# dzufferey/round

Hardware: AMD Instinct MI355X
Metric: checked process-rounds/sec (node), OTR n=64 w/ invariants; % HBM peak (higher is better)
Workload: dtype int32

## Files before the change

round_amd/csrc/psg_api.hip:

```cpp
#include <hip/hip_runtime.h>

#include <algorithm>
#include <cstdio>
#include <cstdlib>
#include <cstring>
#include <new>
#include <string>
#include <thread>
#include <utility>
#include <vector>

#include "../../include/psg.h"
#include "psg_device.hpp"
#include "psg_kernels.hpp"

namespace psg {

__global__ void gen_init_kernel(uint64_t inst_begin, uint64_t count, int n, int alg, int V, uint64_t seed,
                                int32_t* out) {
  const uint64_t total = count * (uint64_t)n;
  for (uint64_t e = (uint64_t)blockIdx.x * blockDim.x + threadIdx.x; e < total; e += (uint64_t)gridDim.x * blockDim.x) {
    const uint64_t i = e / (uint64_t)n;
    const int p = (int)(e - i * (uint64_t)n);
    const uint64_t w = rword(seed, inst_begin + i, ROUND_INIT, (uint32_t)p, 0);
// ... 81 lines not shown
  bool init_f64_host = false;
  std::string module_path;
  hipModule_t module = nullptr;
  hipFunction_t native_fn = nullptr;
  hipFunction_t fused_fn = nullptr, fused_x_fn = nullptr;
  int32_t module_alg = 0;
  bool staged = false;
  bool staged_host = false;
  uint64_t staged_begin = 0, staged_count = 0;
  bool ho_loaded = false, ho_has_crash = false;
  bool pop_crash = false;
  uint64_t ho_begin = 0, ho_count = 0;
  uint64_t last_count = 0;
  int grid_max = 0;
  std::string err;
  std::vector<psg_ctx*> subs;
};

static thread_local std::string g_create_err;

static const char* const k_names_otr[] = {"Safety", "Invariant0", "Invariant1", "Invariant2",
                                          "Agreement", "Validity", "Integrity", "Irrevocability"};
static const char* const k_names_lv[] = {"Safety", "Invariant0", "Invariant1", "Agreement",
                                         "Validity", "Integrity", "Irrevocability"};
static const char* const k_names_benor[] = {"Safety", "Invariant0", "Agreement", "Irrevocability", "SafetyPredicate"};
static const char* const k_names_k[] = {"KAgreement", "KValidity"};
static const char* const k_names_eps[] = {"EpsAgreement", "EpsValidity", "SafetyPredicate"};
static const char* const k_names_tpc[] = {"Safety", "Invariant0", "UniformAgreement", "Validity"};
static const char* const k_names_lattice[] = {"Safety", "Invariant0", "Comparability", "DownwardValidity", "UpwardValidity",
                                              "Irrevocability"};
static_assert(std::size(k_names_otr) == kOtrChecks, "k_names_otr and kOtrChecks disagree");
static_assert(std::size(k_names_lv) == kLvChecks, "k_names_lv and kLvChecks disagree");
static_assert(std::size(k_names_benor) == kBenOrChecks, "k_names_benor and kBenOrChecks disagree");
static_assert(std::size(k_names_k) == kKAgreeChecks, "k_names_k and kKAgreeChecks disagree");
static_assert(std::size(k_names_eps) == kEpsilonChecks, "k_names_eps and kEpsilonChecks disagree");
static_assert(std::size(k_names_tpc) == kTpcChecks, "k_names_tpc and kTpcChecks disagree");
static_assert(std::size(k_names_lattice) == kLatticeChecks, "k_names_lattice and kLatticeChecks disagree");

struct CheckNames {
  const char* const* name;
  int count;
  constexpr CheckNames() : name(nullptr), count(0) {}
  template <int N>
  constexpr CheckNames(const char* const (&a)[N]) : name(a), count(N) {}
};

struct AlgRow {
  const char* class_name;
  CheckNames checks;
  void (*defaults)(psg_config& cfg, int n);
  const char* (*invalid)(const psg_config& cfg);
  hipError_t (*launch)(const KArgs& a, int W, int grid, hipStream_t s);
  const void* (*kernel)(int W);
};

static const char* need_value_range(const psg_config& c) { return c.value_range < 1 ? "value_range must be >= 1" : nullptr; }

static void lv_defaults(psg_config& c, int n) {
  c.value_range = (1 << 15) - 1;
  c.sched.drop_log2 = 4;
  c.sched.good_p32 = 0;
  c.sched.crash_fmax = (n - 1) / 2;
}

static void crash_stop_defaults(psg_config& c, int rounds, int fmax) {
  c.param = 2;
  c.rounds = rounds;
  c.value_range = 1000000;
  c.sched.drop_log2 = 0;
  c.sched.good_p32 = 0;
  c.sched.crash_fmax = fmax;
}

static const char* otr_invalid(const psg_config& c) {
  if (const char* m = need_value_range(c)) return m;
  return c.param < 1 ? "OTR needs afterDecision >= 1" : nullptr;
}

static const AlgRow k_algs[] = {
    {},
    {"example.OTR", k_names_otr, [](psg_config& c, int) { c.param = 2;  }, otr_invalid,
     launch_otr, otr_kernel_ptr},
    {"example.LastVoting", k_names_lv, lv_defaults, need_value_range, launch_lv, lv_kernel_ptr},
    {"example.FloodMin", k_names_k, [](psg_config& c, int) { crash_stop_defaults(c, 4, 2); },
     [](const psg_config& c) {
       if (const char* m = need_value_range(c)) return m;
       return c.param < 0 ? "FloodMin needs f >= 0" : nullptr;
     },
     launch_floodmin, floodmin_kernel_ptr},
    {"example.KSetAgreement", k_names_k, [](psg_config& c, int) { crash_stop_defaults(c, 16, 1); },
     [](const psg_config& c) {
       if (const char* m = need_value_range(c)) return m;
       return c.param < 1 ? "KSetAgreement needs k >= 1" : nullptr;
     },
     launch_kset, kset_kernel_ptr},
    {"example.BenOr", k_names_benor,
     [](psg_config& c, int n) {
       c.rounds = 64;
       c.value_range = 2;
       c.sched.drop_log2 = 2;
       c.sched.good_p32 = 0;
       c.sched.ho_min = n / 2;
     },
     [](const psg_config&) -> const char* { return nullptr; }, launch_benor, benor_kernel_ptr},
    {"example.OTR2", k_names_otr, [](psg_config& c, int) { c.param = 2;  }, otr_invalid,
     launch_otr2, otr2_kernel_ptr},
    {"example.ShortLastVoting", k_names_k,
     [](psg_config& c, int n) {
       lv_defaults(c, n);
       c.rounds = 30;
     },
     need_value_range, launch_slv, slv_kernel_ptr},
    {"example.KSetEarlyStopping", k_names_k,
     [](psg_config& c, int) {
       crash_stop_defaults(c, 3, 2);
       c.param2 = 2;
     },
     [](const psg_config& c) {
       if (const char* m = need_value_range(c)) return m;
       return c.param < 0 || c.param2 < 1 ? "KSetEarlyStopping needs t >= 0 and k >= 1" : nullptr;
     },
     launch_kset_es, kset_es_kernel_ptr},
    {"example.EpsilonConsensus", k_names_eps,
     [](psg_config& c, int n) {
       c.param = 1;
       c.real_param = 0.1;
       c.rounds = 12;
       c.sched.drop_log2 = 4;
       c.sched.good_p32 = 0;
       c.sched.ho_min = n - 2;
     },
     [](const psg_config& c) {
       return c.param < 1 || !(c.real_param > 0.0) ? "EpsilonConsensus needs f >= 1 and epsilon > 0" : nullptr;
     },
     launch_epsilon, epsilon_kernel_ptr},
    {"example.TwoPhaseCommit", k_names_tpc,
     [](psg_config& c, int n) {
       c.param = 0;
       c.rounds = 3;
       c.value_range = 2 * n;
       c.sched.drop_log2 = 6;
       c.sched.good_p32 = 0;
     },
     [](const psg_config& c) {
       if (const char* m = need_value_range(c)) return m;
       return c.param < 0 || c.param >= c.n ? "TwoPhaseCommit needs 0 <= coord < n" : nullptr;
     },
     launch_tpc, tpc_kernel_ptr},
    {"example.LatticeAgreement", k_names_lattice,
     [](psg_config& c, int) {
       c.rounds = 8;
       c.value_range = 16;
       c.sched.drop_log2 = 2;
       c.sched.good_p32 = 0;
     },
     [](const psg_config& c) -> const char* {
       return c.value_range < 1 || c.value_range > 31 ? "LatticeAgreement needs 1 <= value_range <= 31" : nullptr;
     },
     launch_lattice, lattice_kernel_ptr},
// ... 346 lines not shown
    sc.batch_capacity = (cfg->batch_capacity + nd - 1) / nd;
    psg_ctx* sub = nullptr;
    const int rc = psg_create(&sub, &sc);
    if (rc) {
      g_create_err = "device " + std::to_string(cfg->devices[d]) + ": " + g_create_err;
      psg_destroy(c);
      return rc;
    }
    c->subs.push_back(sub);
  }
  *out = c;
  return PSG_OK;
}

int psg_create(psg_ctx** out, const psg_config* cfg) {
  if (!out) return PSG_EINVAL;
  *out = nullptr;
  std::string m;
  int rc = validate(cfg, m);
  if (rc) { g_create_err = m; return rc; }
  if (cfg->n_devices > 0) return create_multi(out, cfg);
  int ndev = 0;
  hipError_t e = hipGetDeviceCount(&ndev);
  if (e != hipSuccess || ndev <= 0) { g_create_err = "no HIP device"; return PSG_ENODEV; }
  if (cfg->device < 0 || cfg->device >= ndev) { g_create_err = "device ordinal out of range"; return PSG_ENODEV; }
  psg_ctx* c = new (std::nothrow) psg_ctx();
  if (!c) return PSG_ENOMEM;
  c->cfg = *cfg;
  c->W = (cfg->n + 63) / 64;
  c->cap = cfg->batch_capacity;
  auto bail = [&](hipError_t err, const char* what) {
    g_create_err = std::string(what) + ": " + hipGetErrorString(err);
    psg_destroy(c);
    return err == hipErrorOutOfMemory ? PSG_ENOMEM : PSG_EIO;
  };
#define CK(call) do { hipError_t e_ = (call); if (e_ != hipSuccess) return bail(e_, #call); } while (0)
  CK(hipSetDevice(cfg->device));
  CK(hipStreamCreateWithFlags(&c->stream, hipStreamNonBlocking));
  CK(hipEventCreate(&c->ev0));
  CK(hipEventCreate(&c->ev1));
  const uint64_t cells = c->cap * (uint64_t)cfg->n;
  if (cfg->alg == PSG_ALG_EPSILON) {
    CK(c->d_init_f64.grow(cells));
    CK(c->d_dec_f64.grow(cells));
  } else {
    CK(c->d_init.grow(cells));
  }
  CK(c->d_dec.grow(cells));
  CK(c->d_dround.grow(cells));
  CK(c->d_inst.grow(c->cap));
  CK(c->d_counters.grow(NCOUNTERS_ALLOC));
  if (cfg->alg == PSG_ALG_KSET && c->W > 1)
    CK(c->d_hand.grow(65 * c->cap + (cells + 1) / 2));
  int per_cu = 0;
  CK(hipOccupancyMaxActiveBlocksPerMultiprocessor(&per_cu, alg_row(cfg->alg)->kernel(c->W), threads_per_block(c->W), 0));
  hipDeviceProp_t prop;
  CK(hipGetDeviceProperties(&prop, cfg->device));
  if (per_cu < 1) per_cu = 1;
  c->grid_max = prop.multiProcessorCount * per_cu;
#undef CK
  *out = c;
  return PSG_OK;
}

static int multi_load_inputs(psg_ctx* c, uint64_t inst_begin, uint64_t count, const int32_t* host_init,
                             const double* host_f64, bool f64) {
  if (count > c->cap) return fail(c, PSG_ERANGE, "inst_count exceeds batch_capacity");
  const uint64_t n = (uint64_t)c->cfg.n, nd = c->subs.size();
  const int rc = par_subs(c, [&](size_t d) {
    uint64_t off, m;
    split(count, nd, d, off, m);
    return f64 ? psg_load_inputs_f64(c->subs[d], inst_begin + off, m, host_f64 ? host_f64 + off * n : nullptr)
               : psg_load_inputs(c->subs[d], inst_begin + off, m, host_init ? host_init + off * n : nullptr);
  });
  if (rc) return rc;
  set_staged(c, inst_begin, count, f64 ? host_f64 != nullptr : host_init != nullptr);
  return PSG_OK;
}

int psg_load_inputs(psg_ctx* c, uint64_t inst_begin, uint64_t count, const int32_t* host_init) {
  if (!c) return PSG_EINVAL;
  if (!c->subs.empty()) {
    if (c->cfg.alg == PSG_ALG_EPSILON && host_init)
      return fail(c, PSG_EINVAL, "EpsilonConsensus takes Double inputs: use psg_load_inputs_f64");
    return multi_load_inputs(c, inst_begin, count, host_init, nullptr, c->cfg.alg == PSG_ALG_EPSILON);
  }
  if (count > c->cap) return fail(c, PSG_ERANGE, "inst_count exceeds batch_capacity");
  if (c->cfg.alg == PSG_ALG_EPSILON) {
    if (host_init) return fail(c, PSG_EINVAL, "EpsilonConsensus takes Double inputs: use psg_load_inputs_f64");
    return psg_load_inputs_f64(c, inst_begin, count, nullptr);
  }
  HIPCHK(c, hipSetDevice(c->cfg.device));
  const uint64_t cells = count * (uint64_t)c->cfg.n;
  if (host_init) {
    HIPCHK(c, hipMemcpyAsync(c->d_init, host_init, sizeof(int32_t) * cells, hipMemcpyHostToDevice, c->stream));
  } else {
    HIPCHK(c, launch_gen_init(inst_begin, count, c->cfg.n, c->cfg.alg, c->cfg.value_range, c->cfg.seed, c->d_init,
                              c->stream));
  }
  HIPCHK(c, hipStreamSynchronize(c->stream));
  set_staged(c, inst_begin, count, host_init != nullptr);
  return PSG_OK;
}

int psg_load_inputs_f64(psg_ctx* c, uint64_t inst_begin, uint64_t count, const double* host_init) {
  if (!c) return PSG_EINVAL;
  if (c->cfg.alg != PSG_ALG_EPSILON) return fail(c, PSG_EINVAL, "Double inputs are for EpsilonConsensus only");
  if (!c->subs.empty()) return multi_load_inputs(c, inst_begin, count, nullptr, host_init, true);
// ... 826 lines not shown
```

round_amd/csrc/psg_device.hpp:

```cpp
#pragma once

#ifndef __HIPCC_RTC__
#include <hip/hip_runtime.h>
#include <stdint.h>
#else
using __hip_internal::int8_t;
using __hip_internal::int16_t;
using __hip_internal::int32_t;
using __hip_internal::int64_t;
using __hip_internal::uint8_t;
using __hip_internal::uint16_t;
using __hip_internal::uint32_t;
using __hip_internal::uint64_t;
#define INT32_MIN (-2147483647 - 1)
#define INT32_MAX 2147483647
#define INT64_MIN (-9223372036854775807LL - 1)
#define INT64_MAX 9223372036854775807LL
#endif

#include "../../include/psg.h"

#define PSG_DEV __device__ __forceinline__

namespace psg {

template <int K>
struct Slot {
  static constexpr int value = K;
};

struct KArgs {
  uint64_t inst_begin;
  uint64_t count;
  const uint64_t* ids;
  const int32_t* init;
  int32_t* out_decision;
  uint8_t* out_dround;
  psg_instance_summary* out_inst;
  psg_process_record* out_rec;
  unsigned long long* counters;
  uint64_t seed;
  const double* init_f64;
  double* out_dec_f64;
  double* out_rec_f64;
  double real_param;
  int32_t* trace;
  uint32_t trace_fields;
  int32_t n, R, V, param, param2, variant, tiebreak;
  uint32_t drop_log2, good_p32;
  int32_t good_min, crash_fmax, ho_min;
  uint32_t self_bit;
  const uint64_t* ho_in;
  const int32_t* crash_in;
  uint64_t ho_base;
  uint64_t init_base;
  uint64_t* hand_hdr;
  uint64_t* hand_meta;
  int32_t* hand_dec;
};

PSG_DEV uint64_t instance_id(const KArgs& a, uint64_t i) { return a.ids ? a.ids[i] : a.inst_begin + i; }
PSG_DEV uint64_t init_row(const KArgs& a, uint64_t i, uint64_t inst) { return a.ids ? inst - a.init_base : i; }
PSG_DEV int32_t init_x(const KArgs& a, uint64_t i, uint64_t inst, int pid) {
#if defined(__HIP_DEVICE_COMPILE__)
  asm volatile("" : "+v"(pid));
#endif
  return a.init[init_row(a, i, inst) * (uint64_t)a.n + (uint64_t)pid];
}

struct VmArgs {
  const int32_t* code;
  const int32_t* slot_entry;
  const int32_t* slot_flags;
  int32_t n_slots, term_entry, n_words;
  const int32_t* trace;
  uint64_t count;
  int32_t n, R;
  psg_instance_summary* out_inst;
  unsigned long long* counters;
  int32_t* err;
};

struct PopArgs {
  uint64_t* ho;
  const uint64_t* src;
  int32_t* init;
  const int32_t* src_init;
  const uint32_t* parent;
  const uint8_t* op;
  uint64_t count;
  int n, R, W;
  uint64_t seed;
  uint32_t gen, flips;
  int32_t min_size;
  uint32_t self_bit;
  uint32_t keep[4];
  int32_t V;
  uint32_t redraw;
  int init_kind;
  int32_t* crash;
  const int32_t* src_crash;
  uint64_t* partial;
  const uint64_t* src_partial;
  int32_t fmax;
  uint32_t partial_p[4];
  uint32_t t_move, t_add, t_drop;
  int32_t live_kind, live_rounds, phase, coord;
  int32_t live_at[PSG_POP_MAX_LIVE];
};
struct LiveArgs {
  const uint64_t* ho;
  uint8_t* live;
  uint64_t count;
  int n, R, W;
  int32_t kind, phase, coord;
};
enum { POP_INIT_VALUE = 0, POP_INIT_COIN = 1, POP_INIT_VOTE = 2, POP_INIT_SET = 3 };

#ifndef PSG_PHASE_TIMERS
#define PSG_PHASE_TIMERS 0
#endif
enum { C_FAIL = 0, C_DECIDED = PSG_MAX_CHECKS, C_DIGEST = PSG_MAX_CHECKS + 1,
       C_ACTIVE = PSG_MAX_CHECKS + 2,
       C_LIVE = PSG_MAX_CHECKS + 3,
       C_HIST = PSG_MAX_CHECKS + 4,
       NCOUNTERS = C_HIST + PSG_MAX_ROUNDS + 2,
       C_QUEUE = NCOUNTERS, NQUEUES = 8, QUEUE_STRIDE = 16, NQUEUE_REGIONS = 2,
       C_TIMER = C_QUEUE + NQUEUE_REGIONS * NQUEUES * QUEUE_STRIDE, NTIMERS = 8, NSTAMP_WAVES = 16384,
       T_RT_SUM = NTIMERS, T_RT_MIN = NTIMERS + 1, T_RT_MAX = NTIMERS + 2, T_WAVES = NTIMERS + 3,
       T_STAMPS = NTIMERS + 4,
       NTIMER_SLOTS = PSG_PHASE_TIMERS ? T_STAMPS + 2 * NSTAMP_WAVES : 0, NCOUNTERS_ALLOC = C_TIMER + NTIMER_SLOTS };

struct PhaseTimers {
#if PSG_PHASE_TIMERS
  uint64_t last, rt0, acc[NTIMERS];
  PSG_DEV void start() {
    for (int j = 0; j < NTIMERS; ++j) acc[j] = 0;
    rt0 = __builtin_amdgcn_s_memrealtime();
    last = __builtin_amdgcn_s_memtime();
  }
  PSG_DEV void mark(int j) {
#if PSG_PHASE_TIMERS == 1
    const uint64_t t = __builtin_amdgcn_s_memtime();
    acc[j] += t - last;
    last = t;
#endif
  }
  PSG_DEV void add(int j, uint64_t v) {
#if PSG_PHASE_TIMERS == 2
    acc[j] += v;
#endif
  }
  PSG_DEV void flush(unsigned long long* g, int lane) {
    const uint64_t rt1 = __builtin_amdgcn_s_memrealtime();
    if (lane == 0) {
      for (int j = 0; j < NTIMERS; ++j) atomicAdd(&g[C_TIMER + j], (unsigned long long)acc[j]);
      atomicAdd(&g[C_TIMER + T_RT_SUM], (unsigned long long)(rt1 - rt0));
      atomicMax(&g[C_TIMER + T_RT_MIN], (unsigned long long)~rt0);
      atomicMax(&g[C_TIMER + T_RT_MAX], (unsigned long long)rt1);
      atomicAdd(&g[C_TIMER + T_WAVES], 1ull);
      const uint32_t wave = blockIdx.x * (blockDim.x >> 6) + (threadIdx.x >> 6);
      if (wave < NSTAMP_WAVES) {
        g[C_TIMER + T_STAMPS + 2 * wave] = rt0;
        g[C_TIMER + T_STAMPS + 1 + 2 * wave] = rt1;
      }
    }
  }
#else
  PSG_DEV void start() {}
  PSG_DEV void mark(int) {}
  PSG_DEV void add(int, uint64_t) {}
  PSG_DEV void flush(unsigned long long*, int) {}
#endif
};

constexpr uint32_t ROUND_INIT = 0xFFFFFFFFu;
constexpr uint32_t ROUND_CRASH = 0xFFFFFFFEu;
constexpr uint32_t PID_GLOBAL = 0xFFFFu;
constexpr uint32_t COIN_TAG = 0x80000000u;

struct U4 { uint32_t x, y, z, w; };

PSG_DEV uint32_t xor3(uint32_t a, uint32_t b, uint32_t c) {
#if defined(__HIP_DEVICE_COMPILE__)
  return __builtin_amdgcn_bitop3_b32(a, b, c, 0x96);
#else
  return a ^ b ^ c;
#endif
}

#ifndef PSG_PHILOX_OPAQUE_KEYS
#define PSG_PHILOX_OPAQUE_KEYS 0
#endif
#ifndef PSG_PHILOX_MAD64
#define PSG_PHILOX_MAD64 2
#endif
#if PSG_PHILOX_MAD64 && defined(__HIP_DEVICE_COMPILE__)
PSG_DEV uint64_t mul64_mad(uint32_t a, uint32_t b) {
  uint64_t r;
#if PSG_PHILOX_MAD64 == 2
  asm("v_mad_u64_u32 %0, vcc, %1, %2, 0" : "=v"(r) : "v"(a), "v"(b) : "vcc");
#else
  uint64_t cy;
  asm("v_mad_u64_u32 %0, %1, %2, %3, 0" : "=v"(r), "=s"(cy) : "v"(a), "v"(b));
#endif
  return r;
}
#define PSG_MUL64(r, a, b) ((r) == 0 ? (uint64_t)(a) * (b) : mul64_mad((a), (b)))
#else
#define PSG_MUL64(r, a, b) ((uint64_t)(a) * (b))
#endif
PSG_DEV U4 philox10(uint32_t c0, uint32_t c1, uint32_t c2, uint32_t c3, uint32_t k0, uint32_t k1) {
#if PSG_PHILOX_OPAQUE_KEYS && defined(__HIP_DEVICE_COMPILE__)
  asm volatile("" : "+s"(k0), "+s"(k1));
#endif
#pragma unroll
  for (int r = 0; r < 10; ++r) {
    const uint64_t p0 = PSG_MUL64(r, 0xD2511F53u, c0);
    const uint64_t p1 = PSG_MUL64(r, 0xCD9E8D57u, c2);
    const uint32_t n0 = xor3((uint32_t)(p1 >> 32), c1, k0);
    const uint32_t n2 = xor3((uint32_t)(p0 >> 32), c3, k1);
    c1 = (uint32_t)p1;
    c3 = (uint32_t)p0;
    c0 = n0;
    c2 = n2;
    k0 += 0x9E3779B9u;
    k1 += 0xBB67AE85u;
  }
  return U4{c0, c1, c2, c3};
}

PSG_DEV uint64_t rword(uint64_t seed, uint64_t inst, uint32_t round, uint32_t ctr3base, uint32_t j) {
  U4 o = philox10((uint32_t)inst, (uint32_t)(inst >> 32), round, ctr3base + ((j >> 1) << 16), (uint32_t)seed,
                  (uint32_t)(seed >> 32));
  return (j & 1u) ? ((uint64_t)o.z | ((uint64_t)o.w << 32)) : ((uint64_t)o.x | ((uint64_t)o.y << 32));
}

struct WordStream {
  uint64_t seed, inst;
  uint32_t round, base;
  int32_t cur;
  uint64_t lo, hi;
  PSG_DEV WordStream(uint64_t s, uint64_t i, uint32_t r, uint32_t b) : seed(s), inst(i), round(r), base(b), cur(-1), lo(0), hi(0) {}
  PSG_DEV uint64_t word(uint32_t j) {
    const int32_t s = (int32_t)(j >> 1);
    if (s != cur) {
      U4 o = philox10((uint32_t)inst, (uint32_t)(inst >> 32), round, base + ((uint32_t)s << 16), (uint32_t)seed,
                      (uint32_t)(seed >> 32));
      lo = (uint64_t)o.x | ((uint64_t)o.y << 32);
      hi = (uint64_t)o.z | ((uint64_t)o.w << 32);
      cur = s;
    }
    return (j & 1u) ? hi : lo;
  }
};

PSG_DEV uint32_t mulhi32(uint32_t a, uint32_t b) { return __umulhi(a, b); }

PSG_DEV int32_t tpc_vote(uint32_t w, uint32_t V) { return mulhi32(w, V) != 0u ? 1 : 0; }

PSG_DEV int32_t lattice_init(uint32_t w, uint32_t U) {
  const uint32_t v = mulhi32(w, U * U);
  return (int32_t)((1u << (v / U)) | (1u << (v % U)));
}

PSG_DEV bool java_first_boolean(uint64_t s) {
  const uint64_t mult = 0x5DEECE66DULL, mask = (1ULL << 48) - 1;
  uint64_t seed = (s ^ mult) & mask;
  seed = (seed * mult + 0xBULL) & mask;
  return (seed >> 47) != 0;
}

PSG_DEV uint32_t scala_improve(uint32_t h) {
  uint32_t x = h + ~(h << 9);
  x ^= (x >> 14);
  x += (x << 4);
  x ^= (x >> 10);
  return x;
}

PSG_DEV uint64_t champ_key(uint32_t h, int depth) {
  uint64_t key = 0;
// ... 505 lines not shown
      return v;
    }
  }
};

template <int W, bool XHO = false>
struct Sched {
  uint64_t seed, inst;
  Mask<W> full;
  int32_t crash_round;
  bool crash_on;
  int good_min, ho_min, V;
  uint32_t drop, good_p32, self_bit;
  int nproc;
  const uint64_t* hop;

  PSG_DEV void setup(const KArgs& args, uint64_t i, int pid, bool valid) {
    hop = nullptr;
    nproc = args.n;
    if constexpr (XHO) {
      const uint64_t row = i - args.ho_base;
      hop = args.ho_in + row * (uint64_t)args.R * (uint64_t)args.n * W;
      seed = args.seed;
      inst = i;
      V = args.V;
      drop = 0;
      good_p32 = 0;
      self_bit = 0;
      ho_min = -1;
      full = mfull<W>(args.n);
      crash_on = false;
      good_min = 0;
      crash_round = (args.crash_in && valid) ? args.crash_in[row * (uint64_t)args.n + pid] : -1;
      return;
    }
    seed = args.seed;
    inst = i;
    V = args.V;
    drop = args.drop_log2;
    good_p32 = args.good_p32;
    self_bit = args.self_bit;
    ho_min = args.ho_min;
    full = mfull<W>(args.n);
    crash_on = args.crash_fmax >= 0;
    good_min = args.good_min >= 0 ? args.good_min : (2 * args.n) / 3;
    crash_round = -1;
    if (crash_on && valid) {
      const uint64_t w0 = rword(seed, i, ROUND_CRASH, PID_GLOBAL, 0);
      const uint64_t w1 = rword(seed, i, ROUND_CRASH, PID_GLOBAL, 1);
      crash_round = crash_of(args, i, (uint32_t)pid, w0, w1);
    }
  }

  PSG_DEV static int32_t crash_of(const KArgs& args, uint64_t i, uint32_t pid, uint64_t w0, uint64_t w1) {
    const uint32_t f = mulhi32((uint32_t)w0, (uint32_t)args.crash_fmax + 1u);
    const uint32_t am = (uint32_t)(w0 >> 32) | 1u;
    const uint32_t off = (uint32_t)w1;
    const uint32_t n = (uint32_t)args.n;
    const bool pow2 = (n & (n - 1)) == 0;
    const uint32_t pos = pow2 ? ((am * pid + off) & (n - 1)) : ((pid + off % n) % n);
    if (pos >= f) return -1;
    return (int32_t)mulhi32((uint32_t)rword(args.seed, i, ROUND_CRASH, pid, 0), (uint32_t)args.R);
  }

  PSG_DEV int32_t init_value(int pid, int alg) const {
    const uint64_t w = rword(seed, inst, ROUND_INIT, (uint32_t)pid, 0);
    if (alg == PSG_ALG_BENOR) return (int32_t)((uint32_t)w & 1u);
    if (alg == PSG_ALG_TPC) return tpc_vote((uint32_t)w, (uint32_t)V);
    if (alg == PSG_ALG_LATTICE) return lattice_init((uint32_t)w, (uint32_t)V);
    return 1 + (int32_t)mulhi32((uint32_t)w, (uint32_t)V);
  }

  PSG_DEV bool coin(int k, int pid) const {
    return java_first_boolean(rword(seed, inst, (uint32_t)k, COIN_TAG | (uint32_t)pid, 0));
  }

  uint64_t good_mask;
  int good_base;
  Mask<W> good_set;

  PSG_DEV void prep_good(int kbase, int lane, int R) {
    good_base = kbase;
    good_mask = 0;
    if (good_p32 == 0) return;
    const int k = kbase + lane;
    WordStream ws(seed, inst, (uint32_t)k, PID_GLOBAL);
    const bool good = k < R && (uint32_t)ws.word(0) < good_p32;
    Mask<W> s = full;
    if (good && drop > 0) {
#pragma unroll
      for (int w = 0; w < W; ++w) {
        uint64_t m = ~0ull;
        for (uint32_t i = 0; i < drop; ++i) m &= ws.word(1u + (uint32_t)w * drop + i);
        s.w[w] &= ~m;
      }
      if (mpopc(s) <= good_min) s = full;
    }
    good_set = s;
    good_mask = __builtin_amdgcn_ballot_w64(good);
  }

  PSG_DEV bool good_round(int k, int lane, int R, Mask<W>& s) {
    if (good_p32 == 0) return false;
    if (k - good_base >= 64) prep_good(k, lane, R);
    const int off = k - good_base;
    const bool good = (good_mask >> off) & 1ull;
// ... 50 lines not shown
      dm[w] = ~0ull;
      hf[w] = ~0ull;
    }
    constexpr bool kSkip = SKIP && W > 1;
    if constexpr (kSkip) {
      if (__builtin_expect(drop == 0 && crash, 0)) {
        {
#pragma unroll
          for (int sc2 = 0; 2 * sc2 < W; ++sc2) {
            if (!((cw >> (2 * sc2)) & 3u)) continue;
            const U4 o = philox10((uint32_t)inst, (uint32_t)(inst >> 32), k, pid + ((uint32_t)sc2 << 16),
                                  (uint32_t)seed, (uint32_t)(seed >> 32));
            hf[2 * sc2] = (uint64_t)o.x | ((uint64_t)o.y << 32);
            if (2 * sc2 + 1 < W) hf[2 * sc2 + 1] = (uint64_t)o.z | ((uint64_t)o.w << 32);
          }
        }
        return;
      }
    }
    draw_words<kSkip>(k, pid, j0, j1, nd, cw, dm, hf);
  }

  PSG_DEV Mask<W> assemble(int pid, bool good, const Mask<W>& goodS, const Mask<W>& CB, const Mask<W>& CN,
                           const uint64_t (&dm)[W], const uint64_t (&hf)[W]) const {
    Mask<W> base;
#pragma unroll
    for (int w = 0; w < W; ++w) {
      base.w[w] = good ? goodS.w[w] : (drop > 0 ? full.w[w] & ~dm[w] : full.w[w]);
      if (crash_on) base.w[w] &= ~(CB.w[w] | (CN.w[w] & ~hf[w]));
    }
    if (self_bit) mset(base, pid);
    if (ho_min >= 0 && mpopc(base) <= ho_min) base = full;
    return base;
  }

  template <bool SKIP = true>
  PSG_DEV Mask<W> ho(int k, int pid, bool good, const Mask<W>& goodS, const Mask<W>& CB, const Mask<W>& CN) const {
    if constexpr (XHO) {
      Mask<W> m = mzero<W>();
      if (pid < nproc) {
        const uint64_t* q = hop + ((uint64_t)k * (uint64_t)nproc + (uint64_t)pid) * W;
#pragma unroll
        for (int w = 0; w < W; ++w) m.w[w] = __builtin_nontemporal_load(q + w) & full.w[w];
      }
      return m;
    }
    uint64_t dm[W], hf[W];
    uint32_t cw = 0;
#pragma unroll
    for (int w = 0; w < W; ++w) cw |= CN.w[w] ? 1u << w : 0u;
    draw<SKIP>((uint32_t)k, (uint32_t)pid, good, crash_on && cw != 0u, dm, hf, cw);
    return assemble(pid, good, goodS, CB, CN, dm, hf);
  }
};

template <int W, bool XHO>
PSG_DEV Mask<W> ho_select(const Sched<W, XHO>& sc, int k, int pid, bool good, const Mask<W>& goodS, const Mask<W>& CB,
                       const Mask<W>& CN) {
  if constexpr (XHO) {
    return sc.ho(k, pid, good, goodS, CB, CN);
  } else {
    uint64_t dm[W], hf[W];
    uint32_t cw = 0;
#pragma unroll
    for (int w = 0; w < W; ++w) cw |= CN.w[w] ? 1u << w : 0u;
    sc.draw((uint32_t)k, (uint32_t)pid, good, sc.crash_on && cw != 0u, dm, hf, cw);
    const uint64_t self = sc.self_bit ? 1ull << (pid & 63) : 0ull;
    Mask<W> base;
#pragma unroll
    for (int w = 0; w < W; ++w) {
      base.w[w] = good ? goodS.w[w] : (sc.drop > 0 ? sc.full.w[w] & ~dm[w] : sc.full.w[w]);
      if (sc.crash_on) base.w[w] &= ~(CB.w[w] | (CN.w[w] & ~hf[w]));
      base.w[w] |= (pid >> 6) == w ? self : 0ull;
    }
    if (sc.ho_min >= 0 && mpopc(base) <= sc.ho_min) base = sc.full;
    return base;
  }
}

template <int W>
struct CrashSets {
  int32_t cr[W];
  PSG_DEV void prep(Grp<W>& g, int32_t* lds, int32_t my_crash_round) {
    if constexpr (W == 1) {
      cr[0] = my_crash_round;
    } else {
      lds[g.pid] = g.valid ? my_crash_round : -1;
      __syncthreads();
#pragma unroll
      for (int w = 0; w < W; ++w) cr[w] = lds[w * 64 + g.lane];
    }
  }
  PSG_DEV void sets(Grp<W>& g, int k, Mask<W>& CB, Mask<W>& CN) const {
    if constexpr (W == 1) {
      CB = g.ballot_any((uint32_t)cr[0] < (uint32_t)k);
      CN = g.ballot_any(cr[0] == k);
    } else {
#pragma unroll
      for (int w = 0; w < W; ++w) {
        CB.w[w] = __builtin_amdgcn_ballot_w64((uint32_t)cr[w] < (uint32_t)k);
        CN.w[w] = __builtin_amdgcn_ballot_w64(cr[w] == k);
      }
    }
  }
};

template <int W, bool XHO>
struct Inst {
  uint64_t id;
  Sched<W, XHO> sc;
  CrashSets<W> cs;
  PSG_DEV void begin(Grp<W>& g, const KArgs& a, uint64_t i, int32_t* crl) {
    begin_front(g, a, i, crl);
    sc.prep_good(0, g.lane, a.R);
  }
  PSG_DEV void begin_front(Grp<W>& g, const KArgs& a, uint64_t i, int32_t* crl) {
    id = instance_id(a, i);
    sc.setup(a, id, g.pid, g.valid);
    if (sc.crash_on) cs.prep(g, crl, sc.crash_round);
  }
  PSG_DEV int32_t x0(const Grp<W>& g, const KArgs& a, uint64_t i, int alg) const {
    if (!g.valid) return 0;
    return a.init ? init_x(a, i, id, g.pid) : sc.init_value(g.pid, alg);
  }
};

struct GoodFront {
  static constexpr int kRows = 8, kRounds = 4, kLate = 32;
  static constexpr uint64_t kNone = 1ull << 63;
  uint64_t g0 = kNone;
  uint32_t set;
  uint32_t mask;
  int base;

  PSG_DEV static bool pass(const Sched<1, false>& sc, uint64_t id, uint32_t k, int lane, int R, uint64_t& s) {
    const uint32_t c = (uint32_t)lane >> 5;
    const U4 o = philox10((uint32_t)id, (uint32_t)(id >> 32), k, PID_GLOBAL + (c << 16), (uint32_t)sc.seed,
                          (uint32_t)(sc.seed >> 32));
    const uint64_t lo = (uint64_t)o.x | ((uint64_t)o.y << 32);
    const uint64_t hi = (uint64_t)o.z | ((uint64_t)o.w << 32);
    const uint64_t t = sc.drop >= 3 ? (lo & hi) : (sc.drop == 2 ? lo : ~0ull);
    const uint64_t up = (uint64_t)xshfl<32>((uint32_t)t, lane) | ((uint64_t)xshfl<32>((uint32_t)(t >> 32), lane) << 32);
    const bool good = lane < 32 && (int)k < R && o.x < sc.good_p32;
    s = sc.full.w[0];
    if (good && sc.drop > 0) {
      uint64_t m = hi & up;
      for (uint32_t c2 = 2; 2 * c2 <= sc.drop; ++c2) {
        const U4 q = philox10((uint32_t)id, (uint32_t)(id >> 32), k, PID_GLOBAL + (c2 << 16), (uint32_t)sc.seed,
                              (uint32_t)(sc.seed >> 32));
        m &= (uint64_t)q.x | ((uint64_t)q.y << 32);
        if (2 * c2 + 1 <= sc.drop) m &= (uint64_t)q.z | ((uint64_t)q.w << 32);
      }
      s &= ~m;
      if (__builtin_popcountll(s) <= sc.good_min) s = sc.full.w[0];
    }
    return good;
  }

  PSG_DEV void start(const Sched<1, false>& sc, const KArgs& a, uint64_t i, int lane) {
    base = kRounds - kLate;
    if (i - g0 < (uint64_t)kRows) return;
#if defined(__HIP_DEVICE_COMPILE__)
    asm volatile("" : "+v"(lane));
#endif
    g0 = i;
    uint64_t row = i + (uint64_t)(lane & (kRows - 1));
    if (a.ids && row >= a.count) row = a.count - 1;
    uint64_t s;
    const bool good = pass(sc, instance_id(a, row), ((uint32_t)lane >> 3) & (uint32_t)(kRounds - 1), lane, a.R, s);
    set = fold(s, lane);
    mask = (uint32_t)__builtin_amdgcn_ballot_w64(good);
  }
// ... 548 lines not shown
```

round_amd/csrc/psg_kernels.hpp:

```cpp
#pragma once
#ifndef __HIPCC_RTC__
#include <hip/hip_runtime.h>

#include <type_traits>

namespace psg {
struct KArgs;
struct VmArgs;
struct PopArgs;
struct LiveArgs;

template <class R, class F>
R with_w(int W, R bad, F&& f) {
  switch (W) {
    case 1: return f(std::integral_constant<int, 1>());
    case 2: return f(std::integral_constant<int, 2>());
    case 3: return f(std::integral_constant<int, 3>());
    case 4: return f(std::integral_constant<int, 4>());
  }
  return bad;
}

hipError_t launch_otr(const KArgs& a, int W, int grid, hipStream_t s);
hipError_t launch_lv(const KArgs& a, int W, int grid, hipStream_t s);
hipError_t launch_floodmin(const KArgs& a, int W, int grid, hipStream_t s);
hipError_t launch_kset(const KArgs& a, int W, int grid, hipStream_t s);
hipError_t launch_benor(const KArgs& a, int W, int grid, hipStream_t s);
hipError_t launch_otr2(const KArgs& a, int W, int grid, hipStream_t s);
hipError_t launch_slv(const KArgs& a, int W, int grid, hipStream_t s);
hipError_t launch_kset_es(const KArgs& a, int W, int grid, hipStream_t s);
hipError_t launch_epsilon(const KArgs& a, int W, int grid, hipStream_t s);
hipError_t launch_tpc(const KArgs& a, int W, int grid, hipStream_t s);
hipError_t launch_lattice(const KArgs& a, int W, int grid, hipStream_t s);
hipError_t launch_otr_packed(const KArgs& a, int G, hipStream_t s);

const void* otr_kernel_ptr(int W);
const void* lv_kernel_ptr(int W);
const void* floodmin_kernel_ptr(int W);
const void* kset_kernel_ptr(int W);
const void* benor_kernel_ptr(int W);
const void* otr2_kernel_ptr(int W);
const void* slv_kernel_ptr(int W);
const void* kset_es_kernel_ptr(int W);
const void* epsilon_kernel_ptr(int W);
const void* tpc_kernel_ptr(int W);
const void* lattice_kernel_ptr(int W);

hipError_t launch_champ_selftest(const uint64_t* sets, int count, int tiebreak, int32_t* out, hipStream_t s);
hipError_t launch_schedule(const KArgs& a, int W, int grid, uint64_t* ho_out, int32_t* crash_out, hipStream_t s);
hipError_t launch_population(const PopArgs& a, hipStream_t s);
hipError_t launch_population_live(const PopArgs& a, hipStream_t s);
hipError_t launch_population_crash(const PopArgs& a, hipStream_t s);
hipError_t launch_live_predicate(const LiveArgs& a, hipStream_t s);
hipError_t launch_spec_vm(const VmArgs& a, int grid, hipStream_t s);
hipError_t launch_gen_init(uint64_t inst_begin, uint64_t count, int n, int alg, int V, uint64_t seed, int32_t* out,
                           hipStream_t s);
}
#endif
```

round_amd/csrc/psg_otr.hip:

```cpp
#include "psg_device.hpp"
#include "psg_kernels.hpp"

namespace psg {

template <int W>
struct OtrLds {
  int32_t xs[W > 1 ? 64 * W : 1];
  int32_t ds[W > 1 ? 64 * W : 1];
};

template <bool V2>
PSG_DEV int32_t otr_check_thresholds(int n, int lane) {
  int32_t t = -1;
  if (!V2 && lane == 1) t = (2 * n) / 3;
  if (lane == 2) t = n - 1;
  if (lane == PSG_MAX_CHECKS) t = INT32_MAX;
  return t;
}


template <int W, bool V2>
PSG_DEV void otr_check_general(Grp<W>& g, OtrLds<W>& L, const X0Set<W>& X0, Checks& ck, int c, bool has_old, int n,
                               const Mask<W>& full, int32_t x, uint32_t dec01, int32_t decision, uint32_t old01,
                               int32_t old_decision, uint32_t valid01, uint32_t od, uint32_t ox, uint32_t irr01) {
// ... 43 lines not shown
  const bool d0in = same && validity;
  const bool inv0 = V2 ? (term || e0) : ((!anyD || e0) && keep);
  const bool inv1 = V2 ? e1 : (e1 && keep);
  const bool inv2 = V2 ? same : (term && d0in);
  const bool integrity = !anyD || d0in;
  const uint32_t fb = fbit(inv0 || inv1 || inv2, 0) | fbit(inv0, 1) | fbit(inv1, 2) | fbit(inv2, 3) |
                      fbit(same, 4) | fbit(validity, 5) | fbit(integrity, 6) | fbit(irrev, 7);
  ck.record(fb, term, c, g.lane);
}

template <int W, bool V2>
PSG_DEV bool otr_check_settled(Grp<W>& g, OtrLds<W>& L, Checks& ck, int c, int n, int32_t x, uint32_t dec01,
                               int32_t decision, uint32_t valid01, uint32_t od, uint32_t ox, uint32_t irr01,
                               int32_t ckthr) {
  if constexpr (W > 1) {
    L.ds[g.pid] = decision;
    __syncthreads();
  }
  const int32_t p0 = g.bcast(decision, L.ds, 0);
  uint32_t u = (1u - dec01) | od | ne01(decision, p0) | irr01;
  if constexpr (!V2) u |= ox;
  if (g.any((u & valid01) != 0u)) return false;
  const int cnt = mpopc(g.ballot(x == p0));
  if constexpr (W == 1) {
    ck.record_le(cnt, ckthr, c);
  } else {
    const int sthr = (2 * n) / 3;
    ck.record((V2 ? 0u : fbit(cnt > sthr, 1)) | fbit(cnt == n, 2), true, c, g.lane);
  }
  return true;
}

template <int W, bool V2, bool FROZEN = false>
PSG_DEV void otr_check(Grp<W>& g, OtrLds<W>& L, const X0Set<W>& X0, Checks& ck, int c, bool has_old, int n,
                       const Mask<W>& full, int32_t x, uint32_t dec01, int32_t decision, uint32_t old01,
                       int32_t old_decision, uint32_t valid01, uint32_t od, uint32_t ox, int32_t ckthr) {
  const uint32_t irr01 = (has_old && !FROZEN) ? old01 & (1u - (dec01 & eq01(old_decision, decision))) : 0u;
  if (!otr_check_settled<W, V2>(g, L, ck, c, n, x, dec01, decision, valid01, od, ox, irr01, ckthr))
    otr_check_general<W, V2>(g, L, X0, ck, c, has_old, n, full, x, dec01, decision, old01, old_decision, valid01, od,
                             ox, irr01);
}

template <bool V2>
PSG_DEV void otr_check_initial(Grp<1>& g, Checks& ck, int n, int32_t x, uint32_t valid01) {
  const int32_t ref = V2 ? majority_candidate<1>(g, x) : readlane32(x, 0);
  const int cnt = mpopc(g.ballot((valid01 & eq01(x, ref)) != 0u));
  const uint32_t ne = opaque_uniform((uint32_t)(cnt - n)) >> 31;
  uint32_t fb = ne << 2;
  if constexpr (V2) fb |= (opaque_uniform((uint32_t)(cnt - (2 * n) / 3 - 1)) >> 31) << 1;
  else fb |= 1u << 3;
  ck.record(fb, false, 0, g.lane);
}

template <int W, bool V2, bool XHO, class SH = NoHook, bool TR = true>
PSG_DEV void otr_body(const KArgs& a) {
  const bool tracing_on = SH::kFused || (TR && a.trace != nullptr);
  constexpr bool kFront = W == 1 && !XHO && !SH::kFused && !TR;
  __shared__ BlockCounters bc;
  __shared__ uint64_t xb[Grp<W>::kXb];
  __shared__ int32_t crl[W > 1 ? 64 * W : 1];
  __shared__ int64_t red[2 * W];
  __shared__ OtrLds<W> L;
  __shared__ int32_t x0tab[Geometry<W>::kGroups][X0Set<W>::kSlots];
  counters_init(&bc);
  __syncthreads();
  Grp<W> g;
  grp_setup(g, a, xb, red);
  const int grp = W == 1 ? (int)(threadIdx.x >> 6) : 0;
  const int n = a.n;
  const int thr = a.variant == 1 ? n / 2 : (2 * n) / 3;
  const Mask<W> full = mfull<W>(n);
  const uint32_t valid01 = g.valid ? 1u : 0u;
  const int32_t ckthr = W == 1 ? otr_check_thresholds<V2>(n, g.lane) : 0;

  PhaseTimers pt;
  pt.start();
  InstanceQueue<W, 0, W == 1 ? PSG_QUEUE_CHUNK_LANE : 0> Q;
  StepTally tally;
  WaveTally wtally;
  GoodFront gf;
  auto load_x0 = [&](uint64_t ii) -> int32_t {
    if (ii == Q.kDone || !a.init || !g.valid) return 0;
    return a.init[init_row(a, ii, instance_id(a, ii)) * (uint64_t)n + g.pid];
  };
  uint64_t inext = Q.take(a);
  int32_t x0next = load_x0(inext);
  while (inext != Q.kDone) {
    const uint64_t i = inext;
    const int32_t x0host = x0next;
    inext = Q.take(a);
    x0next = load_x0(inext);
    pt.mark(4);
    Inst<W, XHO> in;
    if constexpr (kFront) {
      in.begin_front(g, a, i, crl);
      if (a.good_p32 != 0) gf.start(in.sc, a, i, g.lane);
    } else {
      in.begin(g, a, i, crl);
    }
    Sched<W, XHO>& sc = in.sc;
    int32_t x0 = 0;
    if (g.valid) x0 = a.init ? x0host : sc.init_value(g.pid, PSG_ALG_OTR);
    pt.mark(5);
    X0Set<W> X0;
    if constexpr (W == 1) X0.build_window(g, x0tab[grp], x0, a.V);
    else X0.build(g, x0tab[grp], x0);
    pt.mark(6);
    int32_t x = x0, decision = -1, after = a.param;
    uint32_t od, ox;
    X0.maybe_out01_2(decision, x, od, ox);
    uint32_t dec01 = 0, halted01 = 1u - valid01;
    int32_t dec_val = 0, dec_round = -1, halt_round = -1;
    Checks ck;
    ck.reset();
    typename SH::template State<W> sh(g, grp, n);
    if constexpr (!SH::kFused) {
      if constexpr (W == 1) otr_check_initial<V2>(g, ck, n, x, valid01);
      else otr_check<W, V2>(g, L, X0, ck, 0, false, n, full, x, dec01, decision, 0u, -1, valid01, od, ox, ckthr);
    }
    auto trace = [&](int c, int32_t hs, bool frozen = false) {
      emit_state<W, SH>(sh, g, a, i, c, x, (int32_t)dec01, V2 && !dec01 ? PSG_NONE32 : decision, 0, 0, 0, 0, 0, hs,
                        frozen);
    };
    if (tracing_on) trace(0, n);
    pt.mark(0);

    const bool hs_needed = SH::kFused ? ((SH::kFields >> PSG_FIELD_HOSIZE) & 1u) != 0u
                                      : (TR && a.trace != nullptr && ((a.trace_fields >> PSG_FIELD_HOSIZE) & 1u));
    int32_t live_rounds = 0;
    bool good_read = false;
    int kf = a.R;
    for (int k = 0; k < a.R; ++k) {
      const uint32_t old01 = dec01;
      const int32_t old_decision = decision;
      const Mask<W> act = g.ballot_any(halted01 == 0u);
      int32_t hs = n;
      if (!many(act)) {
        kf = k;
        break;
      }
      {
        live_rounds = k + 1;
        bool settled = false;
        if constexpr (W == 1) {
          if (!hs_needed) {
            const int32_t d0 = readlane32(decision, mfirst(act));
            settled = !g.any_raw(halted01 == 0u && !(dec01 != 0u && decision == d0 && x == d0));
          }
        }
        if (!settled) {
        Mask<W> goodS;
        bool good;
        if constexpr (kFront) good = gf.good_round(sc, i, k, g.lane, a.R, goodS);
        else good = sc.good_round(k, g.lane, a.R, goodS);
        pt.add(4, good ? 1u : 0u);
        pt.add(5, good && !good_read ? 1u : 0u);
        if (PSG_PHASE_TIMERS == 2) good_read = good_read || good;
        Mask<W> CB = mzero<W>(), CN = mzero<W>();
        if (sc.crash_on) in.cs.sets(g, k, CB, CN);
        const Mask<W> M = mand(sc.ho(k, g.pid, good, goodS, CB, CN), act);
        const int32_t msize = mpopc(M);
        if (tracing_on) hs = halted01 ? n : msize;
        const uint32_t upd = (1u - halted01) & gt01(msize, thr);
        if (g.any(upd != 0u)) {
          const int32_t xv = x ^ 0x7FFFFFFF;
          if constexpr (W > 1) {
            L.xs[g.pid] = xv;
            __syncthreads();
          }
          uint64_t best = (uint64_t)(uint32_t)(INT32_MAX ^ 0x7FFFFFFF);
          Mask<W> rem = act, passB = mzero<W>(), passS = mzero<W>();
          int stage = 2;
          if constexpr (W == 1) {
            if (k == 0 && X0.bmode && __builtin_popcountll(X0.bm) > 8) {
              int32_t* cnt = x0tab[grp];
              cnt[g.lane] = 0;
              const uint32_t slot = (uint32_t)(x - X0.lo) & 63u;
              if (!halted01) atomicAdd(&cnt[slot], 1);
              const int32_t h = cnt[slot];
              rem = mand(act, g.ballot_any(h >= 3));
              passB = mand(act, g.ballot_any(h == 2));
              passS = mandn(act, mor(rem, passB));
              stage = 0;
            }
          }
          while (true) {
            while (many(rem)) {
              const int32_t kv = g.bcast(xv, L.xs, mfirst(rem));
              const Mask<W> E = g.ballot_any(xv == kv);
              rem = mandn(rem, E);
              const uint64_t key = ((uint64_t)(uint32_t)mpopc(mand(M, E)) << 32) | (uint32_t)kv;
              best = key > best ? key : best;
            }
            if (stage == 2) break;
            const uint32_t beat = stage == 0 ? 3u : 2u;
            if (!g.any(upd != 0u && (uint32_t)(best >> 32) < beat)) break;
            rem = stage == 0 ? passB : passS;
            ++stage;
          }
          const int32_t best_c = (int32_t)(best >> 32);
          const int32_t best_v = (int32_t)((uint32_t)best ^ 0x7FFFFFFFu);
          x = upd ? best_v : x;
          const uint32_t newdec = upd & gt01(best_c, thr);
          const uint32_t first = newdec & (1u - dec01);
          dec_val = first ? best_v : dec_val;
          dec_round = first ? k : dec_round;
          decision = newdec ? best_v : decision;
          dec01 |= newdec;
          if constexpr (!SH::kFused) X0.maybe_out01_2(decision, x, od, ox);
        }
        }
        const uint32_t ad = (1u - halted01) & dec01;
        after -= (int32_t)ad;
        const uint32_t h = ad & gt01(1, after);
        halt_round = h ? k : halt_round;
        halted01 |= h;
      }
      if constexpr (!SH::kFused)
        otr_check<W, V2>(g, L, X0, ck, k + 1, true, n, full, x, dec01, decision, old01, old_decision, valid01, od, ox, ckthr);
      if (tracing_on) trace(k + 1, hs);
      pt.mark(1);
    }
    for (int k = kf; k < a.R; ++k) {
      if constexpr (!SH::kFused)
        otr_check<W, V2, true>(g, L, X0, ck, k + 1, true, n, full, x, dec01, decision, dec01, decision, valid01, od, ox, ckthr);
      if (tracing_on) trace(k + 1, n, true);
      pt.mark(2);
    }
    pt.add(6, 1u);
    if constexpr (W == 1)
      finish_instance_w1(g, a, i, hook_checks<SH>(sh, ck), hook_slots<SH>(kOtrChecks), dec_val, dec_round, halt_round, x,
                         &bc, &tally, &wtally, live_rounds, &pt);
    else
      finish_instance<W>(g, a, i, hook_checks<SH>(sh, ck), hook_slots<SH>(kOtrChecks), dec_val, dec_round, halt_round, x,
                         &bc, &tally, live_rounds, &pt);
    pt.mark(3);
  }
  pt.flush(a.counters, threadIdx.x & 63);
  tally.flush(&bc);
  if constexpr (W == 1) wtally.flush(&bc, hook_slots<SH>(kOtrChecks));
  __syncthreads();
  counters_flush(&bc, a.counters, hook_slots<SH>(kOtrChecks), a.R);
}

#ifndef PSG_OTR_WPE
#define PSG_OTR_WPE 6
#endif
template <int W, bool V2, bool XHO, class SH = NoHook, bool TR = true>
__global__ void __launch_bounds__(Geometry<W>::kThreads) __attribute__((amdgpu_waves_per_eu(W == 1 ? PSG_OTR_WPE : 1)))
otr_kernel(KArgs a) {
  otr_body<W, V2, XHO, SH, TR>(a);
}

#ifndef PSG_FUSED_MODULE
template <int W, bool V2>
static hipError_t launch_w(const KArgs& a, int grid, hipStream_t s) {
  if (a.ho_in) return launch_grp<W>(otr_kernel<W, V2, true>, a, grid, s);
  if (a.trace) return launch_grp<W>(otr_kernel<W, V2, false>, a, grid, s);
  return launch_grp<W>(otr_kernel<W, V2, false, NoHook, false>, a, grid, s);
}

template <bool V2>
static hipError_t launch_v(const KArgs& a, int W, int grid, hipStream_t s) {
  return with_w(W, hipErrorInvalidValue, [&](auto w) { return launch_w<w(), V2>(a, grid, s); });
}

template <bool V2>
static const void* ptr_v(int W) {
  return with_w(W, (const void*)nullptr, [](auto w) { return (const void*)otr_kernel<w(), V2, false, NoHook, false>; });
}

hipError_t launch_otr(const KArgs& a, int W, int grid, hipStream_t s) { return launch_v<false>(a, W, grid, s); }
hipError_t launch_otr2(const KArgs& a, int W, int grid, hipStream_t s) { return launch_v<true>(a, W, grid, s); }
const void* otr_kernel_ptr(int W) { return ptr_v<false>(W); }
const void* otr2_kernel_ptr(int W) { return ptr_v<true>(W); }

#endif

}
```

Before: 799.5 billion.

## Add specialized OTR kernel for crash-free, ho_min-free seeded schedules

Adds a 'plain' OTR kernel variant, used when the schedule has no crashes and no ho_min. It skips crash-set setup and the general HO assembly, and draws drop masks directly with Philox, pairing two Philox streams for the higher drop levels. It launches with a different waves-per-EU target and sizes the grid from that kernel's occupancy. The risk is a draw sequence that must exactly match the general path's random words, plus more code to maintain. It also adds extra phase timer marks.

```diff
diff --git a/round_amd/csrc/psg_api.hip b/round_amd/csrc/psg_api.hip
--- a/round_amd/csrc/psg_api.hip
+++ b/round_amd/csrc/psg_api.hip
@@ -157,6 +157,7 @@
   const char* (*invalid)(const psg_config& cfg);
   hipError_t (*launch)(const KArgs& a, int W, int grid, hipStream_t s);
   const void* (*kernel)(int W);
+  const void* (*kernel_plain)(int W) = nullptr;
 };
 
 static const char* need_value_range(const psg_config& c) { return c.value_range < 1 ? "value_range must be >= 1" : nullptr; }
@@ -185,7 +186,7 @@
 static const AlgRow k_algs[] = {
     {},
     {"example.OTR", k_names_otr, [](psg_config& c, int) { c.param = 2;  }, otr_invalid,
-     launch_otr, otr_kernel_ptr},
+     launch_otr, otr_kernel_ptr, otr_plain_kernel_ptr},
     {"example.LastVoting", k_names_lv, lv_defaults, need_value_range, launch_lv, lv_kernel_ptr},
     {"example.FloodMin", k_names_k, [](psg_config& c, int) { crash_stop_defaults(c, 4, 2); },
      [](const psg_config& c) {
@@ -209,7 +210,7 @@
      },
      [](const psg_config&) -> const char* { return nullptr; }, launch_benor, benor_kernel_ptr},
     {"example.OTR2", k_names_otr, [](psg_config& c, int) { c.param = 2;  }, otr_invalid,
-     launch_otr2, otr2_kernel_ptr},
+     launch_otr2, otr2_kernel_ptr, otr2_plain_kernel_ptr},
     {"example.ShortLastVoting", k_names_k,
      [](psg_config& c, int n) {
        lv_defaults(c, n);
@@ -662,8 +663,11 @@
   CK(c->d_counters.grow(NCOUNTERS_ALLOC));
   if (cfg->alg == PSG_ALG_KSET && c->W > 1)
     CK(c->d_hand.grow(65 * c->cap + (cells + 1) / 2));
+  const AlgRow* row = alg_row(cfg->alg);
+  const bool plain = row->kernel_plain && plain_schedule(make_args(c));
   int per_cu = 0;
-  CK(hipOccupancyMaxActiveBlocksPerMultiprocessor(&per_cu, alg_row(cfg->alg)->kernel(c->W), threads_per_block(c->W), 0));
+  CK(hipOccupancyMaxActiveBlocksPerMultiprocessor(&per_cu, plain ? row->kernel_plain(c->W) : row->kernel(c->W),
+                                                  threads_per_block(c->W), 0));
   hipDeviceProp_t prop;
   CK(hipGetDeviceProperties(&prop, cfg->device));
   if (per_cu < 1) per_cu = 1;
diff --git a/round_amd/csrc/psg_device.hpp b/round_amd/csrc/psg_device.hpp
--- a/round_amd/csrc/psg_device.hpp
+++ b/round_amd/csrc/psg_device.hpp
@@ -59,6 +59,11 @@
   int32_t* hand_dec;
 };
 
+#ifndef PSG_PLAIN_SCHEDULE
+#define PSG_PLAIN_SCHEDULE 1
+#endif
+inline bool plain_schedule(const KArgs& a) { return PSG_PLAIN_SCHEDULE && a.crash_fmax < 0 && a.ho_min < 0; }
+
 PSG_DEV uint64_t instance_id(const KArgs& a, uint64_t i) { return a.ids ? a.ids[i] : a.inst_begin + i; }
 PSG_DEV uint64_t init_row(const KArgs& a, uint64_t i, uint64_t inst) { return a.ids ? inst - a.init_base : i; }
 PSG_DEV int32_t init_x(const KArgs& a, uint64_t i, uint64_t inst, int pid) {
@@ -126,7 +131,7 @@
        C_HIST = PSG_MAX_CHECKS + 4,
        NCOUNTERS = C_HIST + PSG_MAX_ROUNDS + 2,
        C_QUEUE = NCOUNTERS, NQUEUES = 8, QUEUE_STRIDE = 16, NQUEUE_REGIONS = 2,
-       C_TIMER = C_QUEUE + NQUEUE_REGIONS * NQUEUES * QUEUE_STRIDE, NTIMERS = 8, NSTAMP_WAVES = 16384,
+       C_TIMER = C_QUEUE + NQUEUE_REGIONS * NQUEUES * QUEUE_STRIDE, NTIMERS = 12, NSTAMP_WAVES = 16384,
        T_RT_SUM = NTIMERS, T_RT_MIN = NTIMERS + 1, T_RT_MAX = NTIMERS + 2, T_WAVES = NTIMERS + 3,
        T_STAMPS = NTIMERS + 4,
        NTIMER_SLOTS = PSG_PHASE_TIMERS ? T_STAMPS + 2 * NSTAMP_WAVES : 0, NCOUNTERS_ALLOC = C_TIMER + NTIMER_SLOTS };
@@ -228,6 +233,34 @@
     k1 += 0xBB67AE85u;
   }
   return U4{c0, c1, c2, c3};
+}
+
+PSG_DEV void philox10_pair(uint32_t c0, uint32_t c1, uint32_t c2, uint32_t c3a, uint32_t c3b, uint32_t k0, uint32_t k1,
+                           U4& oa, U4& ob) {
+  uint32_t a0 = c0, a1 = c1, a2 = c2, a3 = c3a, b0 = c0, b1 = c1, b2 = c2, b3 = c3b;
+#pragma unroll
+  for (int r = 0; r < 10; ++r) {
+    const uint64_t pa0 = PSG_MUL64(r, 0xD2511F53u, a0);
+    const uint64_t pb0 = PSG_MUL64(r, 0xD2511F53u, b0);
+    const uint64_t pa1 = PSG_MUL64(r, 0xCD9E8D57u, a2);
+    const uint64_t pb1 = PSG_MUL64(r, 0xCD9E8D57u, b2);
+    const uint32_t na0 = xor3((uint32_t)(pa1 >> 32), a1, k0);
+    const uint32_t nb0 = xor3((uint32_t)(pb1 >> 32), b1, k0);
+    const uint32_t na2 = xor3((uint32_t)(pa0 >> 32), a3, k1);
+    const uint32_t nb2 = xor3((uint32_t)(pb0 >> 32), b3, k1);
+    a1 = (uint32_t)pa1;
+    b1 = (uint32_t)pb1;
+    a3 = (uint32_t)pa0;
+    b3 = (uint32_t)pb0;
+    a0 = na0;
+    b0 = nb0;
+    a2 = na2;
+    b2 = nb2;
+    k0 += 0x9E3779B9u;
+    k1 += 0xBB67AE85u;
+  }
+  oa = U4{a0, a1, a2, a3};
+  ob = U4{b0, b1, b2, b3};
 }
 
 PSG_DEV uint64_t rword(uint64_t seed, uint64_t inst, uint32_t round, uint32_t ctr3base, uint32_t j) {
@@ -839,6 +872,23 @@
     }
   }
 
+  PSG_DEV void setup_plain(const KArgs& args, uint64_t i) {
+    static_assert(!XHO, "a seeded schedule");
+    hop = nullptr;
+    nproc = args.n;
+    seed = args.seed;
+    inst = i;
+    V = args.V;
+    drop = args.drop_log2;
+    good_p32 = args.good_p32;
+    self_bit = args.self_bit;
+    ho_min = -1;
+    full = mfull<W>(args.n);
+    crash_on = false;
+    good_min = args.good_min >= 0 ? args.good_min : (2 * args.n) / 3;
+    crash_round = -1;
+  }
+
   PSG_DEV static int32_t crash_of(const KArgs& args, uint64_t i, uint32_t pid, uint64_t w0, uint64_t w1) {
     const uint32_t f = mulhi32((uint32_t)w0, (uint32_t)args.crash_fmax + 1u);
     const uint32_t am = (uint32_t)(w0 >> 32) | 1u;
@@ -995,6 +1045,51 @@
     draw<SKIP>((uint32_t)k, (uint32_t)pid, good, crash_on && cw != 0u, dm, hf, cw);
     return assemble(pid, good, goodS, CB, CN, dm, hf);
   }
+
+  template <int NW>
+  PSG_DEV uint64_t and_words(uint32_t k, uint32_t pid) const {
+    if constexpr (NW <= 2) {
+      const U4 o = philox10((uint32_t)inst, (uint32_t)(inst >> 32), k, pid, (uint32_t)seed, (uint32_t)(seed >> 32));
+      uint64_t m = (uint64_t)o.x | ((uint64_t)o.y << 32);
+      if constexpr (NW == 2) m &= (uint64_t)o.z | ((uint64_t)o.w << 32);
+      return m;
+    } else {
+      U4 o, q;
+      philox10_pair((uint32_t)inst, (uint32_t)(inst >> 32), k, pid, pid + (1u << 16), (uint32_t)seed,
+                    (uint32_t)(seed >> 32), o, q);
+      uint64_t m = ((uint64_t)o.x | ((uint64_t)o.y << 32)) & ((uint64_t)o.z | ((uint64_t)o.w << 32)) &
+                   ((uint64_t)q.x | ((uint64_t)q.y << 32));
+      if constexpr (NW == 4) m &= (uint64_t)q.z | ((uint64_t)q.w << 32);
+      return m;
+    }
+  }
+
+  PSG_DEV Mask<1> ho_plain(uint32_t k, uint32_t pid, bool good, const Mask<1>& goodS, uint64_t selfw) const {
+    static_assert(W == 1 && !XHO, "the plain draw is the seeded W == 1 kernels'");
+    Mask<1> r;
+    if (good) {
+      r.w[0] = goodS.w[0] | selfw;
+      return r;
+    }
+    uint64_t m;
+    switch (drop) {
+      case 0: m = 0ull; break;
+      case 1: m = and_words<1>(k, pid); break;
+      case 2: m = and_words<2>(k, pid); break;
+      case 3: m = and_words<3>(k, pid); break;
+      case 4: m = and_words<4>(k, pid); break;
+      default:
+        m = ~0ull;
+        for (uint32_t c = 0; 2 * c < drop; ++c) {
+          const U4 o = philox10((uint32_t)inst, (uint32_t)(inst >> 32), k, pid + (c << 16), (uint32_t)seed,
+                                (uint32_t)(seed >> 32));
+          m &= (uint64_t)o.x | ((uint64_t)o.y << 32);
+          if (2 * c + 1 < drop) m &= (uint64_t)o.z | ((uint64_t)o.w << 32);
+        }
+    }
+    r.w[0] = (full.w[0] & ~m) | selfw;
+    return r;
+  }
 };
 
 template <int W, bool XHO>
@@ -1061,6 +1156,10 @@
     id = instance_id(a, i);
     sc.setup(a, id, g.pid, g.valid);
     if (sc.crash_on) cs.prep(g, crl, sc.crash_round);
+  }
+  PSG_DEV void begin_plain(const KArgs& a, uint64_t i) {
+    id = instance_id(a, i);
+    sc.setup_plain(a, id);
   }
   PSG_DEV int32_t x0(const Grp<W>& g, const KArgs& a, uint64_t i, int alg) const {
     if (!g.valid) return 0;
diff --git a/round_amd/csrc/psg_kernels.hpp b/round_amd/csrc/psg_kernels.hpp
--- a/round_amd/csrc/psg_kernels.hpp
+++ b/round_amd/csrc/psg_kernels.hpp
@@ -45,6 +45,8 @@
 const void* epsilon_kernel_ptr(int W);
 const void* tpc_kernel_ptr(int W);
 const void* lattice_kernel_ptr(int W);
+const void* otr_plain_kernel_ptr(int W);
+const void* otr2_plain_kernel_ptr(int W);
 
 hipError_t launch_champ_selftest(const uint64_t* sets, int count, int tiebreak, int32_t* out, hipStream_t s);
 hipError_t launch_schedule(const KArgs& a, int W, int grid, uint64_t* ho_out, int32_t* crash_out, hipStream_t s);
diff --git a/round_amd/csrc/psg_otr.hip b/round_amd/csrc/psg_otr.hip
--- a/round_amd/csrc/psg_otr.hip
+++ b/round_amd/csrc/psg_otr.hip
@@ -119,10 +119,11 @@
   ck.record(fb, false, 0, g.lane);
 }
 
-template <int W, bool V2, bool XHO, class SH = NoHook, bool TR = true>
+template <int W, bool V2, bool XHO, class SH = NoHook, bool TR = true, bool PLAIN = false>
 PSG_DEV void otr_body(const KArgs& a) {
   const bool tracing_on = SH::kFused || (TR && a.trace != nullptr);
   constexpr bool kFront = W == 1 && !XHO && !SH::kFused && !TR;
+  static_assert(!PLAIN || kFront, "the plain-schedule form is a seeded, trace-free W == 1 form");
   __shared__ BlockCounters bc;
   __shared__ uint64_t xb[Grp<W>::kXb];
   __shared__ int32_t crl[W > 1 ? 64 * W : 1];
@@ -139,6 +140,7 @@
   const Mask<W> full = mfull<W>(n);
   const uint32_t valid01 = g.valid ? 1u : 0u;
   const int32_t ckthr = W == 1 ? otr_check_thresholds<V2>(n, g.lane) : 0;
+  const uint64_t selfw = PLAIN && a.self_bit ? 1ull << (g.pid & 63) : 0ull;
 
   PhaseTimers pt;
   pt.start();
@@ -160,7 +162,8 @@
     pt.mark(4);
     Inst<W, XHO> in;
     if constexpr (kFront) {
-      in.begin_front(g, a, i, crl);
+      if constexpr (PLAIN) in.begin_plain(a, i);
+      else in.begin_front(g, a, i, crl);
       if (a.good_p32 != 0) gf.start(in.sc, a, i, g.lane);
     } else {
       in.begin(g, a, i, crl);
@@ -223,10 +226,17 @@
         pt.add(4, good ? 1u : 0u);
         pt.add(5, good && !good_read ? 1u : 0u);
         if (PSG_PHASE_TIMERS == 2) good_read = good_read || good;
-        Mask<W> CB = mzero<W>(), CN = mzero<W>();
-        if (sc.crash_on) in.cs.sets(g, k, CB, CN);
-        const Mask<W> M = mand(sc.ho(k, g.pid, good, goodS, CB, CN), act);
+        pt.mark(8);
+        Mask<W> M;
+        if constexpr (PLAIN) {
+          M = mand(sc.ho_plain((uint32_t)k, (uint32_t)g.pid, good, goodS, selfw), act);
+        } else {
+          Mask<W> CB = mzero<W>(), CN = mzero<W>();
+          if (sc.crash_on) in.cs.sets(g, k, CB, CN);
+          M = mand(sc.ho(k, g.pid, good, goodS, CB, CN), act);
+        }
         const int32_t msize = mpopc(M);
+        pt.mark(9);
         if (tracing_on) hs = halted01 ? n : msize;
         const uint32_t upd = (1u - halted01) & gt01(msize, thr);
         if (g.any(upd != 0u)) {
@@ -265,6 +275,7 @@
             rem = stage == 0 ? passB : passS;
             ++stage;
           }
+          pt.mark(10);
           const int32_t best_c = (int32_t)(best >> 32);
           const int32_t best_v = (int32_t)((uint32_t)best ^ 0x7FFFFFFFu);
           x = upd ? best_v : x;
@@ -283,6 +294,7 @@
         halt_round = h ? k : halt_round;
         halted01 |= h;
       }
+      pt.mark(11);
       if constexpr (!SH::kFused)
         otr_check<W, V2>(g, L, X0, ck, k + 1, true, n, full, x, dec01, decision, old01, old_decision, valid01, od, ox, ckthr);
       if (tracing_on) trace(k + 1, hs);
@@ -319,11 +331,20 @@
   otr_body<W, V2, XHO, SH, TR>(a);
 }
 
+template <bool V2>
+__global__ void __launch_bounds__(Geometry<1>::kThreads) __attribute__((amdgpu_waves_per_eu(7)))
+otr_plain_kernel(KArgs a) {
+  otr_body<1, V2, false, NoHook, false, true>(a);
+}
+
 #ifndef PSG_FUSED_MODULE
 template <int W, bool V2>
 static hipError_t launch_w(const KArgs& a, int grid, hipStream_t s) {
   if (a.ho_in) return launch_grp<W>(otr_kernel<W, V2, true>, a, grid, s);
   if (a.trace) return launch_grp<W>(otr_kernel<W, V2, false>, a, grid, s);
+  if constexpr (W == 1) {
+    if (plain_schedule(a)) return launch_grp<W>(otr_plain_kernel<V2>, a, grid, s);
+  }
   return launch_grp<W>(otr_kernel<W, V2, false, NoHook, false>, a, grid, s);
 }
 
@@ -333,14 +354,17 @@
 }
 
 template <bool V2>
-static const void* ptr_v(int W) {
+static const void* ptr_v(int W, bool plain) {
+  if (W == 1 && plain) return (const void*)otr_plain_kernel<V2>;
   return with_w(W, (const void*)nullptr, [](auto w) { return (const void*)otr_kernel<w(), V2, false, NoHook, false>; });
 }
 
 hipError_t launch_otr(const KArgs& a, int W, int grid, hipStream_t s) { return launch_v<false>(a, W, grid, s); }
 hipError_t launch_otr2(const KArgs& a, int W, int grid, hipStream_t s) { return launch_v<true>(a, W, grid, s); }
-const void* otr_kernel_ptr(int W) { return ptr_v<false>(W); }
-const void* otr2_kernel_ptr(int W) { return ptr_v<true>(W); }
+const void* otr_kernel_ptr(int W) { return ptr_v<false>(W, false); }
+const void* otr2_kernel_ptr(int W) { return ptr_v<true>(W, false); }
+const void* otr_plain_kernel_ptr(int W) { return ptr_v<false>(W, true); }
+const void* otr2_plain_kernel_ptr(int W) { return ptr_v<true>(W, true); }
 
 #endif
 
```

Result: faster. 906.6 billion (median of 6 runs) (+13.4%).
